# a-to-the-5/Simple-MapReduce-Search-Engine-Information-Retrieval-

Measured on AMD Instinct MI355X. Metric: index build GB/s of text (top-10 queries/sec in 'query'), higher is better.
Workload: dtype u8 text / int32 postings / f64 weights

## Files before the change

### simple-mapreduce-search-engine-information-retrieval-_amd/csrc/sme_build.hip

```cpp
#include <hip/hip_runtime.h>
#include <limits.h>
#include <math.h>
#include <stdio.h>
#include <stdlib.h>
#include <string.h>

#include <algorithm>
#include <memory>
#include <chrono>

#include "sme_internal.hpp"
#include "sme_text.hpp"
#include "sme_trec.hpp"

namespace sme {


template <typename B>
__device__ bool doc_tag_valid(const B &t, int64_t p, const char *tag, int tl) {
  int chain = 0;
  int64_t x = p;
  for (;;) {
    int64_t q = -1;
    for (int j = 1; j < tl; j++) {
// ... 3988 lines not shown
    ix->P = P;
    prof.mark("docid_pairs");
  }
  const int tbits = split ? bits_for((uint64_t)std::max<int64_t>(Vw - 1, 1)) : bits_for((uint64_t)std::max<int64_t>(Vi, 1));
  uint32_t *key_s = W[W_T0].as<uint32_t>(P + 1);
  int64_t Pm = P;
  int32_t max_tf = 1;
  bool packed = false;
  int64_t dmin = 0;
  uint32_t F = 0;
  if (ai.v32 != nullptr) {
    max_tf = std::max<int32_t>(1, h_mtf);
    packed = true;
    dmin = ai.dmin;
    F = ai.F;
  } else if (P > 0 && !dup_docno && K == 1) {
    SME_HIP(hipMemsetAsync(mtf, 0, sizeof(unsigned int), st));
    const int h_init[2] = {INT_MAX, INT_MIN};
    SME_HIP(hipMemcpyAsync(dmn, h_init, sizeof h_init, hipMemcpyHostToDevice, st));
    hipLaunchKernelGGL(k_pair_stats, dim3(grid_for(P, 256, 2048)), dim3(256), 0, st, p_val, P, mtf);
    hipLaunchKernelGGL(k_docno_range, dim3(grid_for(nR, 256, 1024)), dim3(256), 0, st, docno, nR, dmn, dmx);
    unsigned int h_m = d2h(mtf, st);
    int h_r[2];
    SME_HIP(hipMemcpyAsync(h_r, dmn, sizeof h_r, hipMemcpyDeviceToHost, st));
    SME_HIP(hipStreamSynchronize(st));
    const uint64_t Fq = (uint64_t)h_m + 1, D = (uint64_t)((int64_t)h_r[1] - (int64_t)h_r[0] + 1);
    max_tf = std::max<int32_t>(1, (int32_t)h_m);
    packed = D * Fq < (1ull << 32) && tbits + bits_for((uint64_t)max_tf) <= 32;
    dmin = h_r[0];
    F = (uint32_t)Fq;
  }
  int32_t *docno_d = nullptr, *tf_d = nullptr;
  int64_t *off = nullptr;
  std::vector<double> early_lut;
  bool weights_fused = false;
  if (packed) {
    uint32_t *v32 = ai.v32;
    if (v32 == nullptr) {
      v32 = reinterpret_cast<uint32_t *>(W[W_T1].as<uint64_t>(P + 1));
      hipLaunchKernelGGL(k_pack_pairs, dim3(grid_for(P)), dim3(256), 0, st, p_val, P, dmin, F, v32);
    }
    uint32_t *v32s = W[W_T2].as<uint32_t>(P + 1);
    docno_d = ix->d_docno_d.as<int32_t>(P + 1);
    tf_d = ix->d_tf_d.as<int32_t>(P + 1);
    uint32_t *rscr = W[W_RADIX].as<uint32_t>(term_sort_scratch(P) / sizeof(uint32_t) + 1);
    double *wf = nullptr;
    if (ix->idf_mode == SME_IDF_REFERENCE && P > 0) {
      early_lut.assign((size_t)max_tf + 1, 0.0);
      for (int i = 1; i <= max_tf; i++) early_lut[(size_t)i] = 1.0 + log((double)i);
      SME_HIP(hipMemcpyAsync(ix->d_lut.as<double>(max_tf + 1), early_lut.data(), early_lut.size() * sizeof(double),
                             hipMemcpyHostToDevice, st));
      wf = ix->d_w.as<double>(P + 1);
      weights_fused = true;
    }
    const double idf_r = log10((double)(std::max<int64_t>(nR, 0) / 1));
    const int sort_bits = cx->opt_sort_bits > 0 ? (int)cx->opt_sort_bits : (Pw > (int64_t(1) << 30) ? 8 : 11);
    key_s = term_sort(p_term, v32, key_s, v32s, sort_nrec, sort_reg, sort_xoff, Pw, tbits, dmin, F, docno_d, tf_d, rscr,
                      st, wf ? (const double *)ix->d_lut.p : nullptr, idf_r, wf, sort_bits, xw, P);
    off = ix->d_off.as<int64_t>(Vi + 1);
    SME_HIP(hipMemsetAsync(off, 0, (Vi + 1) * sizeof(int64_t), st));
    if (!split) {
      hipLaunchKernelGGL(k_term_offsets<false>, dim3(grid_for(P)), dim3(256), 0, st, key_s, P, off, Vi);
    } else {
      hipLaunchKernelGGL(k_term_offsets<true>, dim3(grid_for(P)), dim3(256), 0, st, key_s, P, off, Vi);
      hipLaunchKernelGGL(k_docid_off, dim3(grid_for(Vd)), dim3(256), 0, st, dk, Nd, Vd, (const int64_t *)drank,
                         (const int64_t *)wrank_all, Vw, xw, Pw, off);
      if (Nd > 0)
        hipLaunchKernelGGL(k_docid_place, dim3(grid_for(Nd)), dim3(256), 0, st, dk, dv, Nd, (const int64_t *)drank,
                           (const int64_t *)wrank_all, Vw, xw, off, Pw, dmin, F, docno_d, tf_d, key_s,
                           wf ? (const double *)ix->d_lut.p : nullptr, idf_r, wf);
    }
    SME_CHECK_LAUNCH();
  } else {
    uint64_t *val_s = W[W_T1].as<uint64_t>(P + 1);
    if (P > 0)
      sort_pairs_v64<uint32_t>(p_term, key_s, p_val, val_s, P, tbits, cx->ws[120], cx->ws[121], cx->ws[122], st);
    if (dup_docno && P > 0) {
      uint64_t *ck = W[W_PVAL].as<uint64_t>(P), *ck2 = W[W_T2].as<uint64_t>(P);
      int32_t *tfv = reinterpret_cast<int32_t *>(W[W_PTERM].as<uint32_t>(P)), *tf2 = W[W_T3].as<int32_t>(P);
      hipLaunchKernelGGL(k_dup_keys, dim3(grid_for(P)), dim3(256), 0, st, key_s, val_s, P, ck, tfv);
      int64_t *nout = reinterpret_cast<int64_t *>(cnt + 10);
      reduce_by_key_sum(ck, tfv, P, ck2, tf2, nout, cx->ws[120], cx->ws[121], cx->ws[23], st);
      Pm = d2h(nout, st);
      hipLaunchKernelGGL(k_dup_unpack, dim3(grid_for(Pm)), dim3(256), 0, st, ck2, tf2, Pm, key_s, val_s);
    }
    off = ix->d_off.as<int64_t>(Vi + 1);
    SME_HIP(hipMemsetAsync(off, 0, (Vi + 1) * sizeof(int64_t), st));
    if (Pm > 0) hipLaunchKernelGGL(k_term_offsets<false>, dim3(grid_for(Pm)), dim3(256), 0, st, key_s, Pm, off, Vi);
    docno_d = ix->d_docno_d.as<int32_t>(Pm + 1);
// ... 101 lines not shown
      uint32_t *dv = W[W_T3].as<uint32_t>(PP);
      SME_HIP(hipMemcpyAsync(dv, docno_d, (size_t)PP * sizeof(int32_t), hipMemcpyDeviceToDevice, st));
      sort_pairs<uint64_t>(ck, ck2, dv, reinterpret_cast<uint32_t *>(docno_o), PP, tbits + tfb, cx->ws[122], st);
      hipLaunchKernelGGL(k_composite_tf, dim3(grid_for(PP)), dim3(256), 0, st, ck2, PP, tfmask, tf_o);
    }
    SME_CHECK_LAUNCH();
  }
  prof.mark("sort_tf");

  int32_t *rdn = ix->d_rec_docno.as<int32_t>(nR + 1);
  if (nR > 0 && want_packed && h_drange[1] >= h_drange[0]) {
    SME_HIP(hipMemcpyAsync(rdn, docno, nR * sizeof(int32_t), hipMemcpyDeviceToDevice, st));
    ix->dmin = h_drange[0];
    ix->dmax = h_drange[1];
  } else if (nR > 0) {
    SME_HIP(hipMemcpyAsync(rdn, docno, nR * sizeof(int32_t), hipMemcpyDeviceToDevice, st));
    int *dmn = reinterpret_cast<int *>(cnt + 12), *dmx = dmn + 1;
    const int h_init[2] = {INT_MAX, INT_MIN};
    SME_HIP(hipMemcpyAsync(dmn, h_init, sizeof h_init, hipMemcpyHostToDevice, st));
    hipLaunchKernelGGL(k_docno_range, dim3(grid_for(nR, 256, 1024)), dim3(256), 0, st, docno, nR, dmn, dmx);
    int h_r[2];
    SME_HIP(hipMemcpyAsync(h_r, dmn, sizeof h_r, hipMemcpyDeviceToHost, st));
    SME_HIP(hipStreamSynchronize(st));
    ix->dmin = h_r[0];
    ix->dmax = h_r[1];
  }
  prof.mark("finalize");
  ix->V = Vi;
  ix->Vt = V;
  ix->profile = prof.finish();
  ix->profile.emplace_back("tok_attempts", (float)tok_attempts);
  ix->profile.emplace_back("vocab_attempts", (float)vocab_attempts);
  ix->profile.emplace_back("lt_attempts", (float)rsp.lt_attempts);
  ix_guard.release();
  return ix;
}

__global__ void k_reweight(const int64_t *off, int64_t V, const int32_t *tf, const double *lut, double idf_ref,
                           const int64_t *gdf, int64_t N, const double *idf_by_df, int64_t sdf, const double *idf_by_q,
                           int mode, double *w) {
  const int lane = threadIdx.x & 63;
  const int64_t wpb = blockDim.x / 64;
  for (int64_t t = blockIdx.x * wpb + (threadIdx.x >> 6); t < V; t += (int64_t)gridDim.x * wpb) {
    double idf = idf_ref;
    if (mode != SME_IDF_REFERENCE) {
      int64_t df = gdf ? gdf[t] : off[t + 1] - off[t];
      idf = df <= sdf ? idf_by_df[df] : idf_by_q[N / df];
    }
    for (int64_t p = off[t] + lane; p < off[t + 1]; p += 64) w[p] = __dmul_rn(lut[tf[p]], idf);
  }
}

__global__ void k_reweight_flat(const uint32_t *term_of, const int32_t *tf, int64_t P, const double *lut,
                                const double *idf, double *w) {
  for (int64_t p = blockIdx.x * (int64_t)blockDim.x + threadIdx.x; p < P; p += (int64_t)gridDim.x * blockDim.x)
    w[p] = __dmul_rn(lut[tf[p]], idf[term_of[p]]);
}

void reweight_index(sme_index *ix, int64_t N, const int64_t *d_gdf, hipStream_t st, const uint32_t *d_term_of) {
  auto &W = ix->ctx->ws;
  std::vector<double> lut(ix->max_tf + 1, 0.0);
  for (int i = 1; i <= ix->max_tf; i++) lut[i] = 1.0 + log((double)i);
  const int64_t Nn = std::max<int64_t>(N, 0);
  double idf_ref = log10((double)(Nn / 1));
  int64_t sdf = (int64_t)std::sqrt((double)std::max<int64_t>(Nn, 1)) + 1;
  std::vector<double> by_df(sdf + 1), by_q(Nn / std::max<int64_t>(sdf, 1) + 2);
// ... 26 lines not shown
```

### simple-mapreduce-search-engine-information-retrieval-_amd/csrc/sme_internal.hpp

```cpp
#pragma once
#include <hip/hip_runtime.h>
#include <stdint.h>

#include <memory>
#include <string>
#include <vector>

#include "sme_common.hpp"

struct sme_ctx {
  sme::BufPool pool;
  sme_config cfg{};
  int device = 0;
  hipStream_t own_stream = nullptr;
  hipStream_t aux_stream = nullptr;
  hipEvent_t ev_fork = nullptr, ev_join = nullptr;
  std::vector<hipEvent_t> prof_events;
  sme::DevBuf map_chars, map_off;
  int64_t map_n = 0;
  bool has_map = false;
  sme::DevBuf map_slots;
  uint64_t map_mask = 0;
  bool map_hash_ok = false;
  sme::DevBuf ws[128];
// ... 127 lines not shown
    for (size_t i = 1; i < ev.size(); i++) {
      float ms = 0;
      SME_HIP(hipEventElapsedTime(&ms, ev[i - 1].second, ev[i].second));
      out.emplace_back(ev[i].first, ms);
    }
    float tot = 0;
    SME_HIP(hipEventElapsedTime(&tot, ev.front().second, ev.back().second));
    out.emplace_back("total", tot);
    for (auto &p : ev) pool->push_back(p.second);
    ev.clear();
    return out;
  }
};

struct RecordSpans {
  uint64_t *rs, *re;
  int64_t nR;
  uint64_t *C;
  int64_t nC;
  int lt_attempts;
};
void build_docid_hash(sme_ctx *cx, bool distinct, hipStream_t st);
RecordSpans find_records(sme_ctx *cx, const uint8_t *d_text, uint64_t n, hipStream_t st, Prof *prof);
void split_points(sme_ctx *cx, const uint8_t *d_text, uint64_t n, int world, uint64_t *h_cuts, hipStream_t st);
void number_documents(sme_ctx *cx, const uint8_t *d_text, uint64_t n, hipStream_t st, std::vector<uint8_t> &out);
sme_index *build_index(sme_ctx *cx, const uint8_t *d_text, uint64_t n, hipStream_t st, int job = 0);
void chargram_stage(sme_ctx *cx, sme_index *ix, const int32_t *tstream, int64_t M, int64_t V, const int64_t *term_off,
                    const uint16_t *term_chars, hipStream_t st, Prof *prof);
uint32_t *term_sort(uint32_t *k0, uint32_t *v0, uint32_t *k1, uint32_t *v1, int64_t nrec, const int64_t *reg,
                    const int64_t *xoff, int64_t P, int bits, int64_t dmin, uint32_t F, int32_t *docno, int32_t *tf,
                    uint32_t *counts, hipStream_t st, const double *lut = nullptr, double idf = 0.0,
                    double *w = nullptr, int maxbits = 11, const uint2 *xw = nullptr, int64_t Pout = 0);
size_t term_sort_scratch(int64_t P);
template <typename K>
uint32_t *kv_sort(K *k0, uint32_t *v0, K *k1, uint32_t *v1, int64_t n, int bits, uint32_t *scratch, hipStream_t st,
                  bool keys_out = false);
size_t kv_sort_scratch(int64_t n);
template <typename T>
void excl_scan(const T *in, T *out, int64_t n, DevBuf &scratch, hipStream_t st);
void select_flagged(const uint8_t *flag, int64_t n, int32_t *out, int32_t *d_count, DevBuf &s1, DevBuf &s2,
                    hipStream_t st);
template <typename K>
void sort_pairs(K *keys_in, K *keys_out, uint32_t *vals_in, uint32_t *vals_out, int64_t n, int bits, DevBuf &radix,
                hipStream_t st);
template <typename K>
void sort_pairs_v64(K *keys_in, K *keys_out, const uint64_t *vals_in, uint64_t *vals_out, int64_t n, int bits,
                    DevBuf &ia, DevBuf &ib, DevBuf &radix, hipStream_t st);
template <typename T>
void reduce_max(const T *in, int64_t n, T *d_max, hipStream_t st);
void reduce_by_key_sum(const uint64_t *keys, const int32_t *vals, int64_t n, uint64_t *ukeys, int32_t *sums,
                       int64_t *d_runs, DevBuf &flags, DevBuf &pos, DevBuf &scan, hipStream_t st);
void serialize_index(sme_index *ix, hipStream_t st);
void pack_pieces(sme_index *ix, int world, uint8_t *d_out, uint64_t *sizes, hipStream_t st);
sme_index *merge_pieces(sme_ctx *cx, const uint8_t *d_blobs, const uint64_t *sizes, int np, hipStream_t st);
void reweight_index(sme_index *ix, int64_t N, const int64_t *d_gdf, hipStream_t st,
                    const uint32_t *d_term_of = nullptr);
sme_index *load_records(sme_ctx *cx, const uint8_t *d_records, const uint64_t *part_offsets, int np, hipStream_t st);
void prepare_queries(sme_index *ix, hipStream_t st);
void query_topk(sme_index *ix, const int32_t *d_terms, const int64_t *d_qoff, int nq, int k,
                int32_t *d_out_docno, double *d_out_score, uint32_t *d_out_tie, hipStream_t st, int tie_bits = 0);
void query_topk_java7(sme_index *ix, const int32_t *d_terms, const int64_t *d_qoff, int nq, int k,
                      int32_t *d_out_docno, double *d_out_score, uint32_t *d_out_tie, hipStream_t st);
void tokenize_string(sme_ctx *cx, const uint8_t *h_utf8, size_t n, std::vector<std::vector<uint16_t>> &out,
                     hipStream_t st);
void term_fingerprints(sme_index *ix, uint64_t *d_out, hipStream_t st);
void dfx_pack(sme_ctx *cx, const uint64_t *fp, const int64_t *df, int64_t n, int world, uint64_t *sfp, int64_t *sdf,
// ... 11 lines not shown
```

### simple-mapreduce-search-engine-information-retrieval-_amd/csrc/sme_sort.hip

```cpp
#include <hip/hip_runtime.h>

#include "sme_internal.hpp"

namespace sme {
namespace {

#ifndef SME_RSNT
#define SME_RSNT 512
#endif
constexpr int kRsNT = SME_RSNT;
constexpr int kRsWaves = kRsNT / 64;
constexpr int kRsIPL = 16;
constexpr int kRsTile = kRsNT * kRsIPL;
constexpr int kRsWaveItems = 64 * kRsIPL;
constexpr int kRsMaxBits = 11;
constexpr int kRsMaxBins = 1 << kRsMaxBits;
constexpr int kRsBPT = kRsMaxBins / kRsNT;
constexpr int kRsGroups = 1024;
constexpr int kRsScanSums = 1024;

struct RsGroups {
  int64_t tpg;
  int G;
};
static RsGroups rs_groups(int64_t ntiles) {
  const int64_t tpg = std::max<int64_t>(4, (ntiles + kRsGroups - 1) / kRsGroups);
  const int64_t g = (ntiles + tpg - 1) / tpg;
  return RsGroups{tpg, (int)((g + 15) / 16 * 16)};
}

struct Gather {
  const int64_t *reg, *xoff, *crec;
  int64_t nrec;
};
__device__ __forceinline__ void gather_start(const Gather &g, int64_t x, int64_t &rec, int64_t &nx, int64_t &dl) {
  rec = g.crec[x >> 10];
  nx = g.xoff[rec + 1];
  dl = g.reg[rec] - g.xoff[rec];
}
__device__ __forceinline__ int64_t gather_pos(const Gather &g, int64_t x, int64_t &rec, int64_t &nx, int64_t &dl) {
  while (x >= nx) {
    rec++;
    nx = g.xoff[rec + 1];
    dl = g.reg[rec] - g.xoff[rec];
  }
  return x + dl;
}
constexpr int kGRec = 48;
__device__ __forceinline__ int64_t gather_table(const Gather &g, int64_t x0, int lane, int64_t *gx, int64_t *gdl) {
  const int64_t rec0 = g.crec[x0 >> 10];
  const int64_t r = rec0 + lane;
// ... 2 lines not shown
    gdl[lane] = r < g.nrec ? g.reg[r] - g.xoff[r] : 0;
  }
  if (lane == 0) gx[kGRec] = rec0 + kGRec <= g.nrec ? g.xoff[rec0 + kGRec] : INT64_MAX;
  __builtin_amdgcn_fence(__ATOMIC_SEQ_CST, "wavefront");
  __builtin_amdgcn_wave_barrier();
  return rec0;
}
__device__ __forceinline__ int64_t gather_at(const Gather &g, int64_t x, int &j, const int64_t *gx, const int64_t *gdl,
                                             int64_t rec0) {
  while (j < kGRec - 1 && x >= gx[j + 1]) j++;
  if (x < gx[j + 1]) return x + gdl[j];
  int64_t rec = rec0 + kGRec - 1, nx = g.xoff[rec + 1], dl = g.reg[rec] - g.xoff[rec];
  return gather_pos(g, x, rec, nx, dl);
}
__global__ void k_rs_chunk_rec(const int64_t *__restrict__ xoff, int64_t nrec, int64_t P, int64_t *__restrict__ crec) {
  for (int64_t c = blockIdx.x * (int64_t)blockDim.x + threadIdx.x; (c << 10) < P; c += (int64_t)gridDim.x * blockDim.x) {
    const int64_t x = c << 10;
    int64_t lo = 0, hi = nrec;
    while (hi - lo > 1) {
      const int64_t m = (lo + hi) >> 1;
      if (xoff[m] <= x) lo = m;
      else hi = m;
    }
    crec[c] = lo;
  }
}

__global__ __launch_bounds__(kRsNT) void k_rs_count(const uint32_t *__restrict__ key, int64_t P, int shift,
                                                    int nbins, uint32_t *__restrict__ counts, Gather g) {
  __shared__ uint32_t h[kRsMaxBins];
  const int tid = threadIdx.x;
  for (int b = tid; b < nbins; b += kRsNT) h[b] = 0;
  __syncthreads();
  const int64_t t0 = (int64_t)blockIdx.x * kRsTile;
  const uint32_t mask = (uint32_t)nbins - 1u;
  const int64_t n = min((int64_t)kRsTile, P - t0);
  if (g.reg != nullptr) {
    __shared__ int64_t gx_all[kRsWaves][kGRec + 1], gdl_all[kRsWaves][kGRec];
    const int lane = tid & 63, w = tid >> 6;
    const int64_t wb = t0 + (int64_t)w * kRsWaveItems;
    if (wb < P) {
      const int64_t rec0 = gather_table(g, wb, lane, gx_all[w], gdl_all[w]);
      int j = 0;
      uint32_t kk[kRsIPL];
#pragma unroll
      for (int s = 0; s < kRsIPL; s++) {
        const int64_t x = wb + s * 64 + lane;
        kk[s] = x < P ? key[gather_at(g, x, j, gx_all[w], gdl_all[w], rec0)] : 0u;
      }
#pragma unroll
      for (int s = 0; s < kRsIPL; s++)
        if (wb + s * 64 + lane < P) atomicAdd(&h[(kk[s] >> shift) & mask], 1u);
    }
  } else if (n == kRsTile) {
    const uint4 *k4 = reinterpret_cast<const uint4 *>(key + t0);
#pragma unroll
    for (int i = 0; i < kRsIPL / 4; i++) {
      const uint4 v = k4[i * kRsNT + tid];
      atomicAdd(&h[(v.x >> shift) & mask], 1u);
      atomicAdd(&h[(v.y >> shift) & mask], 1u);
      atomicAdd(&h[(v.z >> shift) & mask], 1u);
      atomicAdd(&h[(v.w >> shift) & mask], 1u);
    }
  } else {
    for (int64_t i = tid; i < n; i += kRsNT) atomicAdd(&h[(key[t0 + i] >> shift) & mask], 1u);
  }
  __syncthreads();
  for (int b = tid; b < nbins; b += kRsNT) counts[(int64_t)blockIdx.x * nbins + b] = h[b];
}

__global__ __launch_bounds__(kRsNT) void k_rs_colsum(const uint32_t *__restrict__ counts, int64_t ntiles, int nbins,
                                                     int64_t tpg, int G, uint32_t *__restrict__ gsum) {
  const int g = blockIdx.x;
  const int64_t ta = (int64_t)g * tpg, tb = min(ntiles, ta + tpg);
  for (int b = threadIdx.x; b < nbins; b += kRsNT) {
    uint32_t s = 0;
    for (int64_t t = ta; t < tb; t++) s += counts[t * nbins + b];
    gsum[(int64_t)b * G + g] = s;
  }
}

__global__ __launch_bounds__(kRsNT) void k_rs_scan(uint32_t *__restrict__ a, int n) {
  __shared__ uint32_t ws[kRsWaves];
  const int tid = threadIdx.x, lane = tid & 63, w = tid >> 6;
  uint32_t carry = 0;
  uint4 x[4];
  auto load = [&](int r0, uint4 *y) {
    const int i0 = r0 + 16 * tid;
#pragma unroll
    for (int c = 0; c < 4; c++) y[c] = i0 < n ? reinterpret_cast<const uint4 *>(a + i0)[c] : make_uint4(0, 0, 0, 0);
  };
  load(0, x);
  for (int r0 = 0; r0 < n; r0 += 16 * kRsNT) {
    const int i0 = r0 + 16 * tid;
    uint32_t s = 0;
#pragma unroll
    for (int c = 0; c < 4; c++) s += x[c].x + x[c].y + x[c].z + x[c].w;
    uint32_t incl = s;
// ... 19 lines not shown
        y.x = run;
        run += x[c].x;
        y.y = run;
        run += x[c].y;
        y.z = run;
        run += x[c].z;
        y.w = run;
        run += x[c].w;
        reinterpret_cast<uint4 *>(a + i0)[c] = y;
      }
    }
    carry += tot;
    __syncthreads();
#pragma unroll
    for (int c = 0; c < 4; c++) x[c] = xn[c];
  }
}

__global__ __launch_bounds__(kRsNT) void k_rs_colscan(uint32_t *__restrict__ counts, int64_t ntiles, int nbins,
                                                      int64_t tpg, int G, const uint32_t *__restrict__ gsum) {
  const int g = blockIdx.x;
  const int64_t ta = (int64_t)g * tpg, tb = min(ntiles, ta + tpg);
  for (int b = threadIdx.x; b < nbins; b += kRsNT) {
    uint32_t run = gsum[(int64_t)b * G + g];
    for (int64_t t = ta; t < tb; t++) {
      const uint32_t c = counts[t * nbins + b];
      counts[t * nbins + b] = run;
      run += c;
    }
  }
}

template <bool LAST>
__global__ __launch_bounds__(kRsNT) void k_rs_scatter(const uint32_t *__restrict__ key, const uint32_t *__restrict__ val,
                                                      int64_t P, int shift, int nbits,
                                                      const uint32_t *__restrict__ offs, uint32_t *__restrict__ okey,
                                                      uint32_t *__restrict__ oval, int32_t *__restrict__ odocno,
                                                      int32_t *__restrict__ otf, int64_t dmin, uint32_t F,
                                                      Gather g, const double *__restrict__ lut, double idf,
                                                      double *__restrict__ ow, const uint2 *__restrict__ xw) {
  __shared__ uint16_t wc[kRsWaves * kRsMaxBins];
  __shared__ uint32_t gd[kRsMaxBins];
  __shared__ uint32_t stage[kRsTile];
  __shared__ uint32_t ws[kRsWaves];
  const int tid = threadIdx.x, lane = tid & 63, w = tid >> 6;
  const int nbins = 1 << nbits;
  const uint32_t mask = (uint32_t)nbins - 1u;
  const int64_t per = (int64_t)(gridDim.x >> 3);
  const int64_t tile = (int64_t)(blockIdx.x & 7) * per + (blockIdx.x >> 3);
  const int64_t t0 = tile * kRsTile;
  if (t0 >= P) return;
  const int n = (int)min((int64_t)kRsTile, P - t0);
  for (int i = tid; i < kRsWaves * kRsMaxBins / 2; i += kRsNT) reinterpret_cast<uint32_t *>(wc)[i] = 0u;
  __syncthreads();
  uint16_t *mine = wc + w * kRsMaxBins;
  const int wb = w * kRsWaveItems;
  const uint64_t lt = (1ull << lane) - 1ull;
  uint32_t k[kRsIPL], v[kRsIPL], pos[kRsIPL];
  if (g.reg != nullptr) {
    __shared__ int64_t gx_all[kRsWaves][kGRec + 1], gdl_all[kRsWaves][kGRec];
    int64_t rec0 = 0;
    if (wb < n) rec0 = gather_table(g, t0 + wb, lane, gx_all[w], gdl_all[w]);
    int j = 0;
#pragma unroll
    for (int s = 0; s < kRsIPL; s++) {
      const int i = wb + s * 64 + lane;
      k[s] = 0u;
      v[s] = 0u;
      if (i < n) {
        const int64_t p = gather_at(g, t0 + i, j, gx_all[w], gdl_all[w], rec0);
        k[s] = key[p];
        v[s] = val[p];
      }
    }
  } else {
#pragma unroll
    for (int s = 0; s < kRsIPL; s++) {
      const int i = wb + s * 64 + lane;
      const bool ok = i < n;
      k[s] = ok ? key[t0 + i] : 0u;
      v[s] = ok ? val[t0 + i] : 0u;
    }
  }
#pragma unroll
  for (int s = 0; s < kRsIPL; s++) {
    const bool ok = wb + s * 64 + lane < n;
    const uint32_t d = (k[s] >> shift) & mask;
    uint64_t peers = (uint64_t)__ballot(ok);
    for (int b = 0; b < nbits; b++) {
      const bool bit = (d >> b) & 1u;
      const uint64_t m = (uint64_t)__ballot(bit);
      peers &= bit ? m : ~m;
    }
    uint32_t r = 0;
    if (ok) {
      const uint32_t c = mine[d];
      r = c + (uint32_t)__popcll(peers & lt);
      if ((peers & lt) == 0) mine[d] = (uint16_t)(c + (uint32_t)__popcll(peers));
    }
    pos[s] = r;
  }
  __syncthreads();
  {
    const int b0 = kRsBPT * tid;
    uint32_t tc[kRsBPT];
    uint32_t s2 = 0;
#pragma unroll
    for (int q = 0; q < kRsBPT; q++) {
      tc[q] = 0;
      if (b0 + q < nbins) {
#pragma unroll
        for (int x = 0; x < kRsWaves; x++) tc[q] += wc[x * kRsMaxBins + b0 + q];
      }
      s2 += tc[q];
    }
    uint32_t incl = s2;
    for (int o = 1; o < 64; o <<= 1) {
      const uint32_t u = __shfl_up(incl, o, 64);
      if (lane >= o) incl += u;
    }
    if (lane == 63) ws[w] = incl;
    __syncthreads();
    uint32_t ex = incl - s2;
    for (int j = 0; j < w; j++) ex += ws[j];
#pragma unroll
    for (int q = 0; q < kRsBPT; q++) {
      if (b0 + q < nbins) {
        uint32_t r = ex;
        gd[b0 + q] = offs[tile * nbins + b0 + q] - r;
#pragma unroll
        for (int x = 0; x < kRsWaves; x++) {
          const uint32_t c = wc[x * kRsMaxBins + b0 + q];
          wc[x * kRsMaxBins + b0 + q] = (uint16_t)r;
          r += c;
        }
      }
      ex += tc[q];
    }
  }
  __syncthreads();
#pragma unroll
  for (int s = 0; s < kRsIPL; s++) {
    if (wb + s * 64 + lane >= n) continue;
    pos[s] += mine[(k[s] >> shift) & mask];
    stage[pos[s]] = k[s];
  }
  __syncthreads();
  uint32_t dst[kRsIPL];
#pragma unroll
  for (int j = 0; j < kRsIPL; j++) {
    const int p = j * kRsNT + tid;
    if (p < n) {
      const uint32_t kk = stage[p];
      dst[j] = gd[(kk >> shift) & mask] + (uint32_t)p;
      if (LAST && xw) {
        const uint2 x = xw[kk];
        dst[j] += x.x;
        okey[dst[j]] = x.y;
      } else {
        okey[dst[j]] = kk;
      }
    }
  }
  __syncthreads();
#pragma unroll
  for (int s = 0; s < kRsIPL; s++)
    if (wb + s * 64 + lane < n) stage[pos[s]] = v[s];
  __syncthreads();
#pragma unroll
  for (int j = 0; j < kRsIPL; j++) {
    const int p = j * kRsNT + tid;
    if (p < n) {
      const uint32_t vv = stage[p];
      if (LAST) {
        odocno[dst[j]] = (int32_t)((int64_t)(vv / F) + dmin);
        otf[dst[j]] = (int32_t)(vv % F);
        if (ow) ow[dst[j]] = __dmul_rn(lut[vv % F], idf);
      } else {
        oval[dst[j]] = vv;
      }
    }
  }
}

template <typename K>
__global__ __launch_bounds__(kRsNT) void k_kv_count(const K *__restrict__ key, int64_t n, int shift, int nbins,
                                                    uint32_t *__restrict__ counts) {
  __shared__ uint32_t h[kRsMaxBins];
  const int tid = threadIdx.x;
  for (int b = tid; b < nbins; b += kRsNT) h[b] = 0;
  __syncthreads();
  const int64_t t0 = (int64_t)blockIdx.x * kRsTile;
  const int m = (int)min((int64_t)kRsTile, n - t0);
  const uint32_t mask = (uint32_t)nbins - 1u;
  for (int i = tid; i < m; i += kRsNT) atomicAdd(&h[(uint32_t)(key[t0 + i] >> shift) & mask], 1u);
  __syncthreads();
  for (int b = tid; b < nbins; b += kRsNT) counts[(int64_t)blockIdx.x * nbins + b] = h[b];
}

template <typename K, bool KEYS>
__global__ __launch_bounds__(kRsNT) void k_kv_scatter(const K *__restrict__ key, const uint32_t *__restrict__ val,
                                                      int64_t n_all, int shift, int nbits,
                                                      const uint32_t *__restrict__ offs, K *__restrict__ okey,
                                                      uint32_t *__restrict__ oval) {
  __shared__ uint16_t wc[kRsWaves * kRsMaxBins];
  __shared__ uint32_t gd[kRsMaxBins];
  __shared__ uint32_t stage[kRsTile];
  __shared__ uint32_t ws[kRsWaves];
  const int tid = threadIdx.x, lane = tid & 63, w = tid >> 6;
  const int nbins = 1 << nbits;
  const uint32_t mask = (uint32_t)nbins - 1u;
  const int64_t per = (int64_t)(gridDim.x >> 3);
// ... 201 lines not shown
  for (int64_t i = blockIdx.x * (int64_t)blockDim.x + threadIdx.x; i < n; i += (int64_t)gridDim.x * blockDim.x)
    v[i] = f[i] ? 1 : 0;
}
__global__ void k_select_scatter(const uint8_t *__restrict__ f, const int64_t *__restrict__ pos, int64_t n,
                                 int32_t *__restrict__ out, int32_t *__restrict__ count) {
  for (int64_t i = blockIdx.x * (int64_t)blockDim.x + threadIdx.x; i < n; i += (int64_t)gridDim.x * blockDim.x) {
    if (f[i]) out[pos[i]] = (int32_t)i;
    if (i == n - 1) *count = (int32_t)(pos[i] + (f[i] ? 1 : 0));
  }
}

void rs_scan(uint32_t *gsum, int64_t n, uint32_t *sums, hipStream_t st) {
  if (n <= 16 * 4 * kRsNT) {
    hipLaunchKernelGGL(k_rs_scan, dim3(1), dim3(kRsNT), 0, st, gsum, (int)n);
    return;
  }
  const int64_t nt = (n + kScTile - 1) / kScTile;
  hipLaunchKernelGGL(k_sc_sums<uint32_t>, dim3((unsigned)nt), dim3(kScNT), 0, st, gsum, n, sums);
  hipLaunchKernelGGL(k_sc_carry<uint32_t>, dim3(1), dim3(kScNT), 0, st, sums, nt);
  hipLaunchKernelGGL(k_sc_apply<uint32_t>, dim3((unsigned)nt), dim3(kScNT), 0, st, gsum, gsum, n, sums);
}

}

uint32_t *term_sort(uint32_t *k0, uint32_t *v0, uint32_t *k1, uint32_t *v1, int64_t nrec, const int64_t *reg,
                    const int64_t *xoff, int64_t P, int bits, int64_t dmin, uint32_t F, int32_t *docno, int32_t *tf,
                    uint32_t *counts, hipStream_t st, const double *lut, double idf, double *w, int maxbits,
                    const uint2 *xw, int64_t Pout) {
  if (P <= 0) return k0;
  if (P > 0xFFFFFFFFll) throw Error(SME_ELIMIT, "term sort of more than 2^32 pairs");
  bits = std::max(bits, 1);
  maxbits = std::min(std::max(maxbits, 1), kRsMaxBits);
  const int npass = (bits + maxbits - 1) / maxbits;
  const int64_t ntiles = (P + kRsTile - 1) / kRsTile;
  const RsGroups rg = rs_groups(ntiles);
  const int64_t tpg = rg.tpg;
  const int G = rg.G;
  uint32_t *gsum = counts + ntiles * kRsMaxBins;
  Gather g0{nullptr, nullptr, nullptr, 0};
  if (reg != nullptr) {
    int64_t *crec = reinterpret_cast<int64_t *>(gsum + kRsMaxBins * kRsGroups + kRsScanSums);
    const int64_t nch = (P + 1023) >> 10;
    hipLaunchKernelGGL(k_rs_chunk_rec, dim3((unsigned)std::min<int64_t>((nch + 255) / 256, 4096)), dim3(256), 0, st,
                       xoff, nrec, P, crec);
    g0 = Gather{reg, xoff, crec, nrec};
  }
  int shift = 0;
  for (int p = 0; p < npass; p++) {
    const Gather g = p == 0 ? g0 : Gather{nullptr, nullptr, nullptr, 0};
#ifdef SME_RS_LOFIRST
    const int nb = (bits - shift) / (npass - p);
#else
    const int nb = (bits - shift + (npass - p) - 1) / (npass - p);
#endif
    const int nbins = 1 << nb;
    const bool last = p == npass - 1;
    hipLaunchKernelGGL(k_rs_count, dim3((unsigned)ntiles), dim3(kRsNT), 0, st, k0, P, shift, nbins, counts, g);
    hipLaunchKernelGGL(k_rs_colsum, dim3(G), dim3(kRsNT), 0, st, counts, ntiles, nbins, tpg, G, gsum);
    rs_scan(gsum, (int64_t)nbins * G, gsum + kRsMaxBins * kRsGroups, st);
    hipLaunchKernelGGL(k_rs_colscan, dim3(G), dim3(kRsNT), 0, st, counts, ntiles, nbins, tpg, G, gsum);
    const unsigned sgrid = (unsigned)(8 * ((ntiles + 7) / 8));
    if (last && xw)
      SME_HIP(hipMemsetAsync(k1, 0xFF, (size_t)Pout * sizeof(uint32_t), st));
    if (last)
      hipLaunchKernelGGL(k_rs_scatter<true>, dim3(sgrid), dim3(kRsNT), 0, st, k0, v0, P, shift, nb, counts,
                         k1, nullptr, docno, tf, dmin, F, g, lut, idf, w, xw);
    else
      hipLaunchKernelGGL(k_rs_scatter<false>, dim3(sgrid), dim3(kRsNT), 0, st, k0, v0, P, shift, nb,
                         counts, k1, v1, nullptr, nullptr, dmin, F, g, nullptr, 0.0, nullptr, nullptr);
    SME_CHECK_LAUNCH();
    std::swap(k0, k1);
    std::swap(v0, v1);
    shift += nb;
  }
  return k0;
}

size_t term_sort_scratch(int64_t P) {
  const int64_t ntiles = (std::max<int64_t>(P, 1) + kRsTile - 1) / kRsTile;
  return (size_t)(ntiles * kRsMaxBins + (int64_t)kRsMaxBins * kRsGroups + kRsScanSums) * sizeof(uint32_t) +
         (size_t)(((std::max<int64_t>(P, 1) + 1023) >> 10) + 1) * sizeof(int64_t);
}
template <typename K>
uint32_t *kv_sort(K *k0, uint32_t *v0, K *k1, uint32_t *v1, int64_t n, int bits, uint32_t *scratch, hipStream_t st,
                  bool keys_out) {
  if (n <= 1) return v0;
  if (n > 0xFFFFFFFFll) throw Error(SME_ELIMIT, "sort of more than 2^32 pairs");
  bits = std::min(std::max(bits, 1), (int)(8 * sizeof(K)));
  const int npass = (bits + kRsMaxBits - 1) / kRsMaxBits;
  const int64_t ntiles = (n + kRsTile - 1) / kRsTile;
  const RsGroups rg = rs_groups(ntiles);
  const int64_t tpg = rg.tpg;
  const int G = rg.G;
  uint32_t *counts = scratch, *gsum = scratch + ntiles * kRsMaxBins;
  int shift = 0;
  for (int p = 0; p < npass; p++) {
    const int nb = (bits - shift + (npass - p) - 1) / (npass - p);
    const int nbins = 1 << nb;
    hipLaunchKernelGGL(k_kv_count<K>, dim3((unsigned)ntiles), dim3(kRsNT), 0, st, k0, n, shift, nbins, counts);
    hipLaunchKernelGGL(k_rs_colsum, dim3(G), dim3(kRsNT), 0, st, counts, ntiles, nbins, tpg, G, gsum);
    rs_scan(gsum, (int64_t)nbins * G, gsum + kRsMaxBins * kRsGroups, st);
    hipLaunchKernelGGL(k_rs_colscan, dim3(G), dim3(kRsNT), 0, st, counts, ntiles, nbins, tpg, G, gsum);
    const unsigned sgrid = (unsigned)(8 * ((ntiles + 7) / 8));
    if (p == npass - 1 && !keys_out)
      hipLaunchKernelGGL((k_kv_scatter<K, false>), dim3(sgrid), dim3(kRsNT), 0, st, k0, v0, n, shift, nb, counts,
                         k1, v1);
    else
      hipLaunchKernelGGL((k_kv_scatter<K, true>), dim3(sgrid), dim3(kRsNT), 0, st, k0, v0, n, shift, nb, counts, k1,
                         v1);
    SME_CHECK_LAUNCH();
    std::swap(k0, k1);
    std::swap(v0, v1);
    shift += nb;
// ... 138 lines not shown
```

Before: 167.8.

## Let radix sort blocks process multiple tiles with carried bin offsets

Restructures the term radix sort so each block in the count and scatter kernels can loop over several consecutive tiles (SME_RS_SUB). Per-bin global offsets are carried in registers across sub-tiles, which shrinks the per-block counts table and the column scan work. The scatter kernel also gains a launch-bounds occupancy hint. With the default of one sub-tile, behaviour is close to before, apart from codegen changes and a new profile counter.

```diff
diff --git a/simple-mapreduce-search-engine-information-retrieval-_amd/csrc/sme_build.hip b/simple-mapreduce-search-engine-information-retrieval-_amd/csrc/sme_build.hip
--- a/simple-mapreduce-search-engine-information-retrieval-_amd/csrc/sme_build.hip
+++ b/simple-mapreduce-search-engine-information-retrieval-_amd/csrc/sme_build.hip
@@ -4044,6 +4044,7 @@
   }
   int32_t *docno_d = nullptr, *tf_d = nullptr;
   int64_t *off = nullptr;
+  int64_t sort_blocks = 0;
   std::vector<double> early_lut;
   bool weights_fused = false;
   if (packed) {
@@ -4067,6 +4068,7 @@
     }
     const double idf_r = log10((double)(std::max<int64_t>(nR, 0) / 1));
     const int sort_bits = cx->opt_sort_bits > 0 ? (int)cx->opt_sort_bits : (Pw > (int64_t(1) << 30) ? 8 : 11);
+    sort_blocks = Pw > 0 ? term_sort_blocks(Pw) : 0;
     key_s = term_sort(p_term, v32, key_s, v32s, sort_nrec, sort_reg, sort_xoff, Pw, tbits, dmin, F, docno_d, tf_d, rscr,
                       st, wf ? (const double *)ix->d_lut.p : nullptr, idf_r, wf, sort_bits, xw, P);
     off = ix->d_off.as<int64_t>(Vi + 1);
@@ -4234,6 +4236,7 @@
   ix->profile.emplace_back("tok_attempts", (float)tok_attempts);
   ix->profile.emplace_back("vocab_attempts", (float)vocab_attempts);
   ix->profile.emplace_back("lt_attempts", (float)rsp.lt_attempts);
+  ix->profile.emplace_back("sort_blocks", (float)sort_blocks);
   ix_guard.release();
   return ix;
 }
diff --git a/simple-mapreduce-search-engine-information-retrieval-_amd/csrc/sme_internal.hpp b/simple-mapreduce-search-engine-information-retrieval-_amd/csrc/sme_internal.hpp
--- a/simple-mapreduce-search-engine-information-retrieval-_amd/csrc/sme_internal.hpp
+++ b/simple-mapreduce-search-engine-information-retrieval-_amd/csrc/sme_internal.hpp
@@ -183,6 +183,7 @@
                     uint32_t *counts, hipStream_t st, const double *lut = nullptr, double idf = 0.0,
                     double *w = nullptr, int maxbits = 11, const uint2 *xw = nullptr, int64_t Pout = 0);
 size_t term_sort_scratch(int64_t P);
+int64_t term_sort_blocks(int64_t P);
 template <typename K>
 uint32_t *kv_sort(K *k0, uint32_t *v0, K *k1, uint32_t *v1, int64_t n, int bits, uint32_t *scratch, hipStream_t st,
                   bool keys_out = false);
diff --git a/simple-mapreduce-search-engine-information-retrieval-_amd/csrc/sme_sort.hip b/simple-mapreduce-search-engine-information-retrieval-_amd/csrc/sme_sort.hip
--- a/simple-mapreduce-search-engine-information-retrieval-_amd/csrc/sme_sort.hip
+++ b/simple-mapreduce-search-engine-information-retrieval-_amd/csrc/sme_sort.hip
@@ -17,6 +17,12 @@
 constexpr int kRsMaxBins = 1 << kRsMaxBits;
 constexpr int kRsBPT = kRsMaxBins / kRsNT;
 constexpr int kRsGroups = 1024;
+#ifndef SME_RS_SUB
+#define SME_RS_SUB 1
+#endif
+constexpr int kTsSub = SME_RS_SUB;
+constexpr int64_t kTsBlockItems = (int64_t)kTsSub * kRsTile;
+static_assert(kTsSub >= 1 && kTsSub <= 64, "SME_RS_SUB");
 constexpr int kRsScanSums = 1024;
 
 struct RsGroups {
@@ -85,38 +91,43 @@
   const int tid = threadIdx.x;
   for (int b = tid; b < nbins; b += kRsNT) h[b] = 0;
   __syncthreads();
-  const int64_t t0 = (int64_t)blockIdx.x * kRsTile;
   const uint32_t mask = (uint32_t)nbins - 1u;
-  const int64_t n = min((int64_t)kRsTile, P - t0);
-  if (g.reg != nullptr) {
-    __shared__ int64_t gx_all[kRsWaves][kGRec + 1], gdl_all[kRsWaves][kGRec];
-    const int lane = tid & 63, w = tid >> 6;
-    const int64_t wb = t0 + (int64_t)w * kRsWaveItems;
-    if (wb < P) {
-      const int64_t rec0 = gather_table(g, wb, lane, gx_all[w], gdl_all[w]);
-      int j = 0;
-      uint32_t kk[kRsIPL];
-#pragma unroll
-      for (int s = 0; s < kRsIPL; s++) {
-        const int64_t x = wb + s * 64 + lane;
-        kk[s] = x < P ? key[gather_at(g, x, j, gx_all[w], gdl_all[w], rec0)] : 0u;
-      }
-#pragma unroll
-      for (int s = 0; s < kRsIPL; s++)
-        if (wb + s * 64 + lane < P) atomicAdd(&h[(kk[s] >> shift) & mask], 1u);
-    }
-  } else if (n == kRsTile) {
-    const uint4 *k4 = reinterpret_cast<const uint4 *>(key + t0);
-#pragma unroll
-    for (int i = 0; i < kRsIPL / 4; i++) {
-      const uint4 v = k4[i * kRsNT + tid];
-      atomicAdd(&h[(v.x >> shift) & mask], 1u);
-      atomicAdd(&h[(v.y >> shift) & mask], 1u);
-      atomicAdd(&h[(v.z >> shift) & mask], 1u);
-      atomicAdd(&h[(v.w >> shift) & mask], 1u);
-    }
-  } else {
-    for (int64_t i = tid; i < n; i += kRsNT) atomicAdd(&h[(key[t0 + i] >> shift) & mask], 1u);
+#pragma unroll
+  for (int sub = 0; sub < kTsSub; sub++) {
+    const int64_t t0 = (int64_t)blockIdx.x * kTsBlockItems + (int64_t)sub * kRsTile;
+    if (t0 >= P) break;
+    const int64_t n = min((int64_t)kRsTile, P - t0);
+    if (g.reg != nullptr) {
+      __shared__ int64_t gx_all[kRsWaves][kGRec + 1], gdl_all[kRsWaves][kGRec];
+      const int lane = tid & 63, w = tid >> 6;
+      const int64_t wb = t0 + (int64_t)w * kRsWaveItems;
+      if (wb < P) {
+        __builtin_amdgcn_wave_barrier();
+        const int64_t rec0 = gather_table(g, wb, lane, gx_all[w], gdl_all[w]);
+        int j = 0;
+        uint32_t kk[kRsIPL];
+#pragma unroll
+        for (int s = 0; s < kRsIPL; s++) {
+          const int64_t x = wb + s * 64 + lane;
+          kk[s] = x < P ? key[gather_at(g, x, j, gx_all[w], gdl_all[w], rec0)] : 0u;
+        }
+#pragma unroll
+        for (int s = 0; s < kRsIPL; s++)
+          if (wb + s * 64 + lane < P) atomicAdd(&h[(kk[s] >> shift) & mask], 1u);
+      }
+    } else if (n == kRsTile) {
+      const uint4 *k4 = reinterpret_cast<const uint4 *>(key + t0);
+#pragma unroll
+      for (int i = 0; i < kRsIPL / 4; i++) {
+        const uint4 v = k4[i * kRsNT + tid];
+        atomicAdd(&h[(v.x >> shift) & mask], 1u);
+        atomicAdd(&h[(v.y >> shift) & mask], 1u);
+        atomicAdd(&h[(v.z >> shift) & mask], 1u);
+        atomicAdd(&h[(v.w >> shift) & mask], 1u);
+      }
+    } else {
+      for (int64_t i = tid; i < n; i += kRsNT) atomicAdd(&h[(key[t0 + i] >> shift) & mask], 1u);
+    }
   }
   __syncthreads();
   for (int b = tid; b < nbins; b += kRsNT) counts[(int64_t)blockIdx.x * nbins + b] = h[b];
@@ -202,152 +213,164 @@
 }
 
 template <bool LAST>
-__global__ __launch_bounds__(kRsNT) void k_rs_scatter(const uint32_t *__restrict__ key, const uint32_t *__restrict__ val,
-                                                      int64_t P, int shift, int nbits,
-                                                      const uint32_t *__restrict__ offs, uint32_t *__restrict__ okey,
-                                                      uint32_t *__restrict__ oval, int32_t *__restrict__ odocno,
-                                                      int32_t *__restrict__ otf, int64_t dmin, uint32_t F,
-                                                      Gather g, const double *__restrict__ lut, double idf,
-                                                      double *__restrict__ ow, const uint2 *__restrict__ xw) {
+__global__ __launch_bounds__(kRsNT, 4) void k_rs_scatter(
+    const uint32_t *__restrict__ key, const uint32_t *__restrict__ val, int64_t P, int shift, int nbits,
+    const uint32_t *__restrict__ offs, uint32_t *__restrict__ okey, uint32_t *__restrict__ oval,
+    int32_t *__restrict__ odocno, int32_t *__restrict__ otf, int64_t dmin, uint32_t F, Gather g,
+    const double *__restrict__ lut, double idf, double *__restrict__ ow, const uint2 *__restrict__ xw) {
   __shared__ uint16_t wc[kRsWaves * kRsMaxBins];
   __shared__ uint32_t gd[kRsMaxBins];
   __shared__ uint32_t stage[kRsTile];
   __shared__ uint32_t ws[kRsWaves];
+  __shared__ int64_t gx_all[kRsWaves][kGRec + 1], gdl_all[kRsWaves][kGRec];
   const int tid = threadIdx.x, lane = tid & 63, w = tid >> 6;
   const int nbins = 1 << nbits;
   const uint32_t mask = (uint32_t)nbins - 1u;
   const int64_t per = (int64_t)(gridDim.x >> 3);
-  const int64_t tile = (int64_t)(blockIdx.x & 7) * per + (blockIdx.x >> 3);
-  const int64_t t0 = tile * kRsTile;
-  if (t0 >= P) return;
-  const int n = (int)min((int64_t)kRsTile, P - t0);
-  for (int i = tid; i < kRsWaves * kRsMaxBins / 2; i += kRsNT) reinterpret_cast<uint32_t *>(wc)[i] = 0u;
-  __syncthreads();
+  const int64_t blk = (int64_t)(blockIdx.x & 7) * per + (blockIdx.x >> 3);
+  const int64_t g0 = blk * kTsBlockItems;
+  if (g0 >= P) return;
   uint16_t *mine = wc + w * kRsMaxBins;
   const int wb = w * kRsWaveItems;
   const uint64_t lt = (1ull << lane) - 1ull;
+  const int b0 = kRsBPT * tid;
+  uint32_t run[kRsBPT];
+#pragma unroll
+  for (int q = 0; q < kRsBPT; q++) run[q] = b0 + q < nbins ? offs[blk * nbins + b0 + q] : 0u;
   uint32_t k[kRsIPL], v[kRsIPL], pos[kRsIPL];
-  if (g.reg != nullptr) {
-    __shared__ int64_t gx_all[kRsWaves][kGRec + 1], gdl_all[kRsWaves][kGRec];
-    int64_t rec0 = 0;
-    if (wb < n) rec0 = gather_table(g, t0 + wb, lane, gx_all[w], gdl_all[w]);
-    int j = 0;
+  auto load = [&](int64_t t0, int il) {
+    const int64_t n = min((int64_t)kRsTile, P - t0);
+    if (g.reg != nullptr) {
+      int64_t rec0 = 0;
+      __builtin_amdgcn_wave_barrier();
+      if (wb < n) rec0 = gather_table(g, t0 + wb, lane, gx_all[w], gdl_all[w]);
+      int j = 0;
+#pragma unroll
+      for (int s = 0; s < kRsIPL; s++) {
+        const int i = il + s * 64;
+        int64_t p = 0;
+        if (i < n) p = gather_at(g, t0 + i, j, gx_all[w], gdl_all[w], rec0);
+        k[s] = i < n ? key[p] : 0u;
+        v[s] = i < n ? val[p] : 0u;
+      }
+    } else {
+#pragma unroll
+      for (int s = 0; s < kRsIPL; s++) {
+        const int i = il + s * 64;
+        const bool ok = i < n;
+        k[s] = ok ? key[t0 + i] : 0u;
+        v[s] = ok ? val[t0 + i] : 0u;
+      }
+    }
+  };
+#pragma unroll 1
+  for (int sub = 0; sub < kTsSub; sub++) {
+    const int64_t t0 = g0 + (int64_t)sub * kRsTile;
+    if (t0 >= P) break;
+    int il = wb + lane, tl = tid;
+    asm volatile("" : "+v"(il), "+v"(tl));
+    const int n = (int)min((int64_t)kRsTile, P - t0);
+    for (int i = tid; i < kRsWaves * kRsMaxBins / 2; i += kRsNT) reinterpret_cast<uint32_t *>(wc)[i] = 0u;
+    __syncthreads();
+    load(t0, il);
 #pragma unroll
     for (int s = 0; s < kRsIPL; s++) {
-      const int i = wb + s * 64 + lane;
-      k[s] = 0u;
-      v[s] = 0u;
-      if (i < n) {
-        const int64_t p = gather_at(g, t0 + i, j, gx_all[w], gdl_all[w], rec0);
-        k[s] = key[p];
-        v[s] = val[p];
-      }
-    }
-  } else {
+      const bool ok = il + s * 64 < n;
+      const uint32_t d = (k[s] >> shift) & mask;
+      uint64_t peers = (uint64_t)__ballot(ok);
+      for (int b = 0; b < nbits; b++) {
+        const bool bit = (d >> b) & 1u;
+        const uint64_t m = (uint64_t)__ballot(bit);
+        peers &= bit ? m : ~m;
+      }
+      uint32_t r = 0;
+      if (ok) {
+        const uint32_t c = mine[d];
+        r = c + (uint32_t)__popcll(peers & lt);
+        if ((peers & lt) == 0) mine[d] = (uint16_t)(c + (uint32_t)__popcll(peers));
+      }
+      pos[s] = r;
+    }
+    __syncthreads();
+    {
+      uint32_t tc[kRsBPT];
+      uint32_t s2 = 0;
+#pragma unroll
+      for (int q = 0; q < kRsBPT; q++) {
+        tc[q] = 0;
+        if (b0 + q < nbins) {
+#pragma unroll
+          for (int x = 0; x < kRsWaves; x++) tc[q] += wc[x * kRsMaxBins + b0 + q];
+        }
+        s2 += tc[q];
+      }
+      uint32_t incl = s2;
+      for (int o = 1; o < 64; o <<= 1) {
+        const uint32_t u = __shfl_up(incl, o, 64);
+        if (lane >= o) incl += u;
+      }
+      if (lane == 63) ws[w] = incl;
+      __syncthreads();
+      uint32_t ex = incl - s2;
+      for (int j = 0; j < w; j++) ex += ws[j];
+#pragma unroll
+      for (int q = 0; q < kRsBPT; q++) {
+        if (b0 + q < nbins) {
+          uint32_t r = ex;
+          gd[b0 + q] = run[q] - r;
+          run[q] += tc[q];
+#pragma unroll
+          for (int x = 0; x < kRsWaves; x++) {
+            const uint32_t c = wc[x * kRsMaxBins + b0 + q];
+            wc[x * kRsMaxBins + b0 + q] = (uint16_t)r;
+            r += c;
+          }
+        }
+        ex += tc[q];
+      }
+    }
+    __syncthreads();
 #pragma unroll
     for (int s = 0; s < kRsIPL; s++) {
-      const int i = wb + s * 64 + lane;
-      const bool ok = i < n;
-      k[s] = ok ? key[t0 + i] : 0u;
-      v[s] = ok ? val[t0 + i] : 0u;
-    }
-  }
-#pragma unroll
-  for (int s = 0; s < kRsIPL; s++) {
-    const bool ok = wb + s * 64 + lane < n;
-    const uint32_t d = (k[s] >> shift) & mask;
-    uint64_t peers = (uint64_t)__ballot(ok);
-    for (int b = 0; b < nbits; b++) {
-      const bool bit = (d >> b) & 1u;
-      const uint64_t m = (uint64_t)__ballot(bit);
-      peers &= bit ? m : ~m;
-    }
-    uint32_t r = 0;
-    if (ok) {
-      const uint32_t c = mine[d];
-      r = c + (uint32_t)__popcll(peers & lt);
-      if ((peers & lt) == 0) mine[d] = (uint16_t)(c + (uint32_t)__popcll(peers));
-    }
-    pos[s] = r;
-  }
-  __syncthreads();
-  {
-    const int b0 = kRsBPT * tid;
-    uint32_t tc[kRsBPT];
-    uint32_t s2 = 0;
-#pragma unroll
-    for (int q = 0; q < kRsBPT; q++) {
-      tc[q] = 0;
-      if (b0 + q < nbins) {
-#pragma unroll
-        for (int x = 0; x < kRsWaves; x++) tc[q] += wc[x * kRsMaxBins + b0 + q];
-      }
-      s2 += tc[q];
-    }
-    uint32_t incl = s2;
-    for (int o = 1; o < 64; o <<= 1) {
-      const uint32_t u = __shfl_up(incl, o, 64);
-      if (lane >= o) incl += u;
-    }
-    if (lane == 63) ws[w] = incl;
-    __syncthreads();
-    uint32_t ex = incl - s2;
-    for (int j = 0; j < w; j++) ex += ws[j];
-#pragma unroll
-    for (int q = 0; q < kRsBPT; q++) {
-      if (b0 + q < nbins) {
-        uint32_t r = ex;
-        gd[b0 + q] = offs[tile * nbins + b0 + q] - r;
-#pragma unroll
-        for (int x = 0; x < kRsWaves; x++) {
-          const uint32_t c = wc[x * kRsMaxBins + b0 + q];
-          wc[x * kRsMaxBins + b0 + q] = (uint16_t)r;
-          r += c;
+      if (il + s * 64 >= n) continue;
+      pos[s] += mine[(k[s] >> shift) & mask];
+      stage[pos[s]] = k[s];
+    }
+    __syncthreads();
+    uint32_t dst[kRsIPL];
+#pragma unroll
+    for (int j = 0; j < kRsIPL; j++) {
+      const int p = j * kRsNT + tl;
+      dst[j] = 0u;
+      if (p < n) {
+        const uint32_t kk = stage[p];
+        dst[j] = gd[(kk >> shift) & mask] + (uint32_t)p;
+        if (LAST && xw) {
+          const uint2 x = xw[kk];
+          dst[j] += x.x;
+          okey[dst[j]] = x.y;
+        } else {
+          okey[dst[j]] = kk;
         }
       }
-      ex += tc[q];
-    }
-  }
-  __syncthreads();
-#pragma unroll
-  for (int s = 0; s < kRsIPL; s++) {
-    if (wb + s * 64 + lane >= n) continue;
-    pos[s] += mine[(k[s] >> shift) & mask];
-    stage[pos[s]] = k[s];
-  }
-  __syncthreads();
-  uint32_t dst[kRsIPL];
-#pragma unroll
-  for (int j = 0; j < kRsIPL; j++) {
-    const int p = j * kRsNT + tid;
-    if (p < n) {
-      const uint32_t kk = stage[p];
-      dst[j] = gd[(kk >> shift) & mask] + (uint32_t)p;
-      if (LAST && xw) {
-        const uint2 x = xw[kk];
-        dst[j] += x.x;
-        okey[dst[j]] = x.y;
-      } else {
-        okey[dst[j]] = kk;
-      }
-    }
-  }
-  __syncthreads();
-#pragma unroll
-  for (int s = 0; s < kRsIPL; s++)
-    if (wb + s * 64 + lane < n) stage[pos[s]] = v[s];
-  __syncthreads();
-#pragma unroll
-  for (int j = 0; j < kRsIPL; j++) {
-    const int p = j * kRsNT + tid;
-    if (p < n) {
-      const uint32_t vv = stage[p];
-      if (LAST) {
-        odocno[dst[j]] = (int32_t)((int64_t)(vv / F) + dmin);
-        otf[dst[j]] = (int32_t)(vv % F);
-        if (ow) ow[dst[j]] = __dmul_rn(lut[vv % F], idf);
-      } else {
-        oval[dst[j]] = vv;
+    }
+    __syncthreads();
+#pragma unroll
+    for (int s = 0; s < kRsIPL; s++)
+      if (il + s * 64 < n) stage[pos[s]] = v[s];
+    __syncthreads();
+#pragma unroll
+    for (int j = 0; j < kRsIPL; j++) {
+      const int p = j * kRsNT + tl;
+      if (p < n) {
+        const uint32_t vv = stage[p];
+        if (LAST) {
+          odocno[dst[j]] = (int32_t)((int64_t)(vv / F) + dmin);
+          otf[dst[j]] = (int32_t)(vv % F);
+          if (ow) ow[dst[j]] = __dmul_rn(lut[vv % F], idf);
+        } else {
+          oval[dst[j]] = vv;
+        }
       }
     }
   }
@@ -615,11 +638,11 @@
   bits = std::max(bits, 1);
   maxbits = std::min(std::max(maxbits, 1), kRsMaxBits);
   const int npass = (bits + maxbits - 1) / maxbits;
-  const int64_t ntiles = (P + kRsTile - 1) / kRsTile;
-  const RsGroups rg = rs_groups(ntiles);
+  const int64_t nblk = term_sort_blocks(P);
+  const RsGroups rg = rs_groups(nblk);
   const int64_t tpg = rg.tpg;
   const int G = rg.G;
-  uint32_t *gsum = counts + ntiles * kRsMaxBins;
+  uint32_t *gsum = counts + nblk * kRsMaxBins;
   Gather g0{nullptr, nullptr, nullptr, 0};
   if (reg != nullptr) {
     int64_t *crec = reinterpret_cast<int64_t *>(gsum + kRsMaxBins * kRsGroups + kRsScanSums);
@@ -638,11 +661,11 @@
 #endif
     const int nbins = 1 << nb;
     const bool last = p == npass - 1;
-    hipLaunchKernelGGL(k_rs_count, dim3((unsigned)ntiles), dim3(kRsNT), 0, st, k0, P, shift, nbins, counts, g);
-    hipLaunchKernelGGL(k_rs_colsum, dim3(G), dim3(kRsNT), 0, st, counts, ntiles, nbins, tpg, G, gsum);
+    hipLaunchKernelGGL(k_rs_count, dim3((unsigned)nblk), dim3(kRsNT), 0, st, k0, P, shift, nbins, counts, g);
+    hipLaunchKernelGGL(k_rs_colsum, dim3(G), dim3(kRsNT), 0, st, counts, nblk, nbins, tpg, G, gsum);
     rs_scan(gsum, (int64_t)nbins * G, gsum + kRsMaxBins * kRsGroups, st);
-    hipLaunchKernelGGL(k_rs_colscan, dim3(G), dim3(kRsNT), 0, st, counts, ntiles, nbins, tpg, G, gsum);
-    const unsigned sgrid = (unsigned)(8 * ((ntiles + 7) / 8));
+    hipLaunchKernelGGL(k_rs_colscan, dim3(G), dim3(kRsNT), 0, st, counts, nblk, nbins, tpg, G, gsum);
+    const unsigned sgrid = (unsigned)(8 * ((nblk + 7) / 8));
     if (last && xw)
       SME_HIP(hipMemsetAsync(k1, 0xFF, (size_t)Pout * sizeof(uint32_t), st));
     if (last)
@@ -659,9 +682,11 @@
   return k0;
 }
 
+int64_t term_sort_blocks(int64_t P) { return (std::max<int64_t>(P, 1) + kTsBlockItems - 1) / kTsBlockItems; }
+
 size_t term_sort_scratch(int64_t P) {
-  const int64_t ntiles = (std::max<int64_t>(P, 1) + kRsTile - 1) / kRsTile;
-  return (size_t)(ntiles * kRsMaxBins + (int64_t)kRsMaxBins * kRsGroups + kRsScanSums) * sizeof(uint32_t) +
+  const int64_t nblk = term_sort_blocks(P);
+  return (size_t)(nblk * kRsMaxBins + (int64_t)kRsMaxBins * kRsGroups + kRsScanSums) * sizeof(uint32_t) +
          (size_t)(((std::max<int64_t>(P, 1) + 1023) >> 10) + 1) * sizeof(int64_t);
 }
 template <typename K>
```

Result: no change. 167.7 (median of 3 runs) (-0.1%).
